# neka-nat/probreg

Hardware: AMD Instinct MI355X
Metric: EM iterations/sec (RigidCPD, N=M=100k fp32) (higher is better)
Workload: dtype f32; 1 GPU; C1 RigidCPD fp32 synthetic N=M=100000 D=3 w=0; window=EM iterations 0..2332 of the registration (state reset after the warm-up steps), collective=none, m=100000, n_local=100000, n_global=100000

## Files before the change

probreg_amd/csrc/cpd.hip:

```cpp
#include <math.h>

#include <algorithm>
#include <cmath>
#include <cstdlib>
#include <cstring>
#include <vector>

#include "cpd_estep.h"
#include "cpd_mstep.h"
#include "cpd_sweeps.h"
#include "morton.h"
#include "small_linalg.h"

namespace {
using prg::block_reduce_store;
using prg::ensure_mompart;
using prg::grid1;
using prg::kBlock;
using prg::kMomComp;
using prg::row_moment_terms;


__global__ __launch_bounds__(kBlock) void k_pack_cloud(const float* __restrict__ in, int64_t n, int dim,
                                                       float4* __restrict__ out, int64_t cap, float pad,
// ... 184 lines not shown
    PRG_HIP(hipMemsetAsync(h->motion.p, 0, 16 * sizeof(unsigned), h->stream));
    return PRG_OK;
}

int morton_permutation(prg_cpd* h, const float* pts_hd, int64_t n, int dim, prg::DevBuf<int>* perm_dev, double* ext2 = nullptr,
                       float* box = nullptr) {
    std::vector<float> host((size_t)n * dim);
    PRG_HIP(hipMemcpy(host.data(), pts_hd, host.size() * sizeof(float), hipMemcpyDefault));
    if (ext2) {
        *ext2 = 0.0;
        for (int k = 0; k < 3; ++k) {
            float lo = INFINITY, hi = -INFINITY;
            for (int64_t i = 0; i < n && k < dim; ++i) {
                lo = std::min(lo, host[(size_t)i * dim + k]);
                hi = std::max(hi, host[(size_t)i * dim + k]);
            }
            if (k >= dim) lo = hi = 0.f;
            *ext2 += (double)(hi - lo) * (double)(hi - lo);
            if (box) {
                box[k] = lo;
                box[3 + k] = hi;
            }
        }
    }
    PRG_HIP(perm_dev->reset(n));
    const std::string& order = prg::cpd_env().spatial_order;
    if (order != "morton" && order != "kd_host") {
        PRG_TRY(prg::ensure_stage(h, (size_t)n * dim * sizeof(float)));
        PRG_HIP(hipMemcpyAsync(h->stage.p, host.data(), host.size() * sizeof(float), hipMemcpyHostToDevice, h->stream));
        return prg::device_kd_order((const float*)h->stage.p, n, dim, perm_dev->p, h->stream);
    }
    const std::vector<int> perm = order == "morton" ? prg::morton_order(host.data(), n, dim) : prg::kd_order(host.data(), n, dim);
    PRG_HIP(hipMemcpy(perm_dev->p, perm.data(), (size_t)n * sizeof(int), hipMemcpyHostToDevice));
    return PRG_OK;
}

}

namespace prg {
int ensure_stage(prg_cpd* h, size_t bytes) {
    if (h->stage.cap >= (int64_t)bytes) return PRG_OK;
    if (h->stage.p) PRG_HIP(hipStreamSynchronize(h->stream));
    PRG_HIP(h->stage.reset((int64_t)bytes));
    return PRG_OK;
}

const CpdEnv& cpd_env() {
    static const CpdEnv env = [] {
        CpdEnv e;
        auto num = [](const char* name, double absent) { const char* v = getenv(name); return v ? atof(v) : absent; };
        auto is_zero = [](const char* name) { const char* v = getenv(name); return v && atoi(v) == 0; };
        e.mfma_seg = getenv("PRG_MFMA_SEG") ? atoi(getenv("PRG_MFMA_SEG")) : 0;
        e.fine_grid_off = is_zero("PRG_MFMA_FINE_GRID");
        e.r_col = num("PRG_ENGINE_RCOL", 0.0);
        e.r_row = num("PRG_ENGINE_RROW", 0.0);
        e.fused_rcol_scale = num("PRG_FUSED_RCOL_SCALE", -1.0);
        e.lean_factor = num("PRG_LEAN_FACTOR", -1.0);
        e.fused_factor = num("PRG_FUSED_FACTOR", -1.0);
        e.owner_off = is_zero("PRG_OWNER_SWEEP");
        e.debug_engine = getenv("PRG_DEBUG_ENGINE") != nullptr;
        if (const char* v = getenv("PRG_SPATIAL_ORDER")) e.spatial_order = v;
        return e;
    }();
    return env;
}

int ensure_engine_state(prg_cpd* h) {
    if (h->eng_dev.p) return PRG_OK;
    PRG_HIP(h->eng_host.ensure(1, kMailboxFlags));
    h->eng_host_dev = h->eng_host.dev;
    PRG_HIP(h->eng_dev.reset(1));
    PRG_HIP(hipMemsetAsync(h->eng_dev.p, 0, sizeof(EngineState), h->stream));
    h->eng_work = h->eng_dev.p->work;
    h->tsum_local = h->eng_dev.p->tsum;
    return PRG_OK;
}
}

extern "C" {

int prg_cpd_create(prg_cpd** out, int device, void* hip_stream) {
    PRG_REQUIRE(out != nullptr, PRG_ERR_INVALID, "prg_cpd_create: out is NULL");
    int count = 0;
    PRG_HIP(hipGetDeviceCount(&count));
    PRG_REQUIRE(device >= 0 && device < count, PRG_ERR_INVALID, "prg_cpd_create: device %d out of range (%d devices)",
                device, count);
    prg::DeviceGuard g(device);
    PRG_REQUIRE(g.ok, PRG_ERR_HIP, "prg_cpd_create: hipSetDevice(%d) failed", device);
    prg_cpd* h = new (std::nothrow) prg_cpd();
    PRG_REQUIRE(h != nullptr, PRG_ERR_NOMEM, "prg_cpd_create: out of host memory");
    h->device = device;
    h->stream = (hipStream_t)hip_stream;
    if (const char* eng = getenv("PRG_DENSE_ENGINE")) h->dense_engine = std::max(0, std::min(2, atoi(eng)));
    if (const char* eng = getenv("PRG_SPARSE_ENGINE")) h->sparse_engine = std::max(0, std::min(2, atoi(eng)));
    if (const char* eng = getenv("PRG_RESID_SWEEP")) h->resid_sweep = atoi(eng) != 0;
    const hipError_t e = h->state.reset(PRG_NMOMENTS + PRG_NPARAMS);
    if (e != hipSuccess) {
        delete h;
        prg::set_error("prg_cpd_create: device allocation failed: %s", hipGetErrorString(e));
        return PRG_ERR_HIP;
    }
    h->moments = h->state.p;
    h->params = h->state.p + PRG_NMOMENTS;
    k_zero_doubles<<<1, 64, 0, h->stream>>>(h->state.p, PRG_NMOMENTS + PRG_NPARAMS);
    *out = h;
    return PRG_OK;
// ... 505 lines not shown
```

probreg_amd/csrc/cpd_estep.hip:

```cpp
#include <math.h>

#include <algorithm>
#include <cmath>

#include "cpd_estep.h"
#include "cpd_sweeps.h"

namespace {
using prg::block_reduce_store;
using prg::grid1;
using prg::kBlock;
using prg::kMomComp;
using prg::row_moment_terms;

constexpr double kLog2e = 1.4426950408889634;

constexpr int kRedBlock = 1024;
__global__ __launch_bounds__(kRedBlock) void k_reduce_partials(const double* __restrict__ part, int nblk, int ncomp,
                                                               double* __restrict__ out, int off) {
    __shared__ double sh[32][33];
    const int c = threadIdx.x & 31, slice = threadIdx.x >> 5;
    double s = 0.0;
    if (c < ncomp)
        for (int b = slice; b < nblk; b += 32) s += part[(int64_t)b * ncomp + c];
// ... 822 lines not shown
    *out = L;
    return PRG_OK;
}
}

namespace {
int ensure_estep_buffers(prg_cpd* h, const EstepLayout& L) {
    PRG_HIP(h->colpart.ensure(L.colpart_elems, L.colpart_elems));
    PRG_HIP(h->rowpart.ensure(L.rowpart_elems, L.rowpart_elems));
    PRG_HIP(h->mompart.ensure(L.mompart_elems, L.mompart_elems));
    if (L.use_queue) PRG_TRY(prg::prepare_queues(h));
    if (L.wgcount_elems > h->wg_cap()) {
        if (h->wgcount.p) PRG_HIP(hipStreamSynchronize(h->stream));
        PRG_HIP(h->wgcount.reset(2 * L.wgcount_elems));
    }
    return PRG_OK;
}

int transform_source(prg_cpd* h, int slot) {
    const double* disp = h->bcpd ? h->W.p : nullptr;
    if (h->nonrigid) PRG_TRY(prg::nonrigid_displacement(h, &disp));
    k_transform_linear<<<(unsigned)prg::ceil_div(h->M, kBlock), kBlock, 0, h->stream>>>(
        h->src4.p, h->z4.p, h->M, h->params, h->motion.p, slot, h->zmeta.p, h->srcw.p, disp, h->zchunk.p);
    return PRG_OK;
}

struct EstepEngines {
    bool use_mfma = false, row_mfma = false;
    bool first = false;
    bool fine = false;
    bool row_lean = false;
    bool fused = false;
    bool col_launched = false;
};

void fill_engine_args(prg_cpd* h, const EstepLayout& L, int slot, EngineArgs* out) {
    const CpdEnv& env = prg::cpd_env();
    EngineArgs ea;
    ea.ext2 = std::max(h->sext2, h->text2);
    ea.r_col_bound = env.r_col > 0.0 ? env.r_col : h->dense_bound > 0.0 ? h->dense_bound : prg::engine_col_bound(h->M, h->N);
    ea.r_col_bound_fused = ea.r_col_bound * fused_lower_bound_scale(L.allow_resid);
    ea.r_row_bound = env.r_row > 0.0 ? env.r_row : prg::engine_row_bound(h->M, h->N, true);
    ea.r_row_bound_full = env.r_row > 0.0 ? env.r_row : prg::engine_row_bound(h->M, h->N, false);
    ea.streamed_col = (double)h->M;
    ea.streamed_row = (double)h->N;
    h->q_first_col = first_queue_unit(ea.r_col_bound, h->N, h->M);
    h->q_first_row = first_queue_unit(ea.r_row_bound, h->M, h->N);
    ea.owned_col = (double)h->N;
    ea.owned_row = (double)h->M;
    ea.work = h->eng_work;
    ea.tsum = h->tsum_local;
    ea.dim = h->D;
    ea.lean_factor = h->lean_factor >= 0.0 ? h->lean_factor : env.lean_factor >= 0.0 ? env.lean_factor : kLeanFactor;
    ea.fused_allowed = L.allow_fused ? 1 : 0;
    ea.resid_allowed = L.allow_resid ? 1 : 0;
    ea.fused_factor = env.fused_factor >= 0.0 ? env.fused_factor : h->fused_factor;
    ea.reset = h->eng.reset ? 1 : 0;
    for (int k = 0; k < 6; ++k) ea.tbox[k] = h->tbox[k];
    ea.slot = slot;
    ea.have_colmin = h->have_colmin ? 1 : 0;
    ea.forced = h->dense_engine >= 2 ? 1 : 0;
    ea.seq = (unsigned)h->estep_count;
    ea.dev = &h->eng_dev.p->decision;
    ea.host = h->eng_host_dev;
    *out = ea;
}

int decide_engines(prg_cpd* h, const EstepLayout& L, int slot, bool cull_seed, hipEvent_t* ev, EstepEngines* out) {
    EstepEngines d;
    *out = d;
    if (!L.mfma_possible || h->eng.mfma_off) {
        if (ev) PRG_HIP(hipEventRecord(ev[1], h->stream));
        return PRG_OK;
    }
    PRG_TRY(prg::ensure_engine_state(h));
    EngineArgs ea;
    fill_engine_args(h, L, slot, &ea);
    h->eng.reset = false;
    prg::launch_chunk_meta_bbox(h, &ea);
    if (ev) PRG_HIP(hipEventRecord(ev[1], h->stream));
    auto seg_col = [&]() { return h->eng.grid_fine && L.seg_col_fine ? L.seg_col_fine : prg::cpd_env().mfma_seg; };
    const bool pred = h->eng.pred_col != 0, pred_fused = L.allow_fused && h->eng.pred_fused != 0;
    const bool vector_grid = !L.use_queue && !L.use_owner;
    if (pred_fused)
        prg::launch_fused_mfma(h, seg_col(), !h->have_colmin, false, ea.dev);
    else if (pred)
        prg::launch_colpass_mfma(h, seg_col(), !h->have_colmin, false, ea.dev, h->mfma_stream && h->eng.pred_fine == 0 && !h->eng.grid_fine);
    else if (vector_grid)
        prg::launch_colpass_cull(h, L.SA, L.segA, cull_seed, ea.dev, L.allow_resid);
    PRG_HIP(hipGetLastError());
    volatile EngineDecision* mb = h->eng_host.p;
    hipError_t werr;
    const bool got = prg::wait_mailbox(&mb->seq, ea.seq, h->stream, &werr);
    PRG_HIP(werr);
    PRG_REQUIRE(got, PRG_ERR_HIP, "prg_cpd_estep: the engine decision never reached the host");
    d.use_mfma = mb->col != 0;
    d.first = mb->first != 0;
    d.row_mfma = mb->row != 0;
    d.fine = mb->fine != 0;
    d.row_lean = d.row_mfma && mb->lean != 0;
    d.fused = L.allow_fused && mb->fused != 0;
    if (!mb->dense) h->eng.mfma_off = true;
    h->eng.grid_fine = !d.first && (double)mb->r_col < 0.9 * (double)h->M;
    if (prg::cpd_env().debug_engine)
        fprintf(stderr, "[engine] sigma2 %.4e nk*ext2 %.1f pairs per owned point col %.0f (bound %.0f) row %.0f (bound %.0f) motion %.3e cmax %.3e nk*width %.1f "
                        "nk*far2 %.1f have_colmin %d -> col %d (first %d, launched ahead: %s) row %d fine %d\n",
                (double)mb->sigma2, (double)mb->nk_ext2, (double)mb->r_col, ea.r_col_bound, (double)mb->r_row, ea.r_row_bound,
                (double)mb->motion, (double)mb->cmax,
                (double)mb->nk_width, (double)mb->nk_far2, (int)h->have_colmin, (int)d.use_mfma, (int)d.first,
                pred == d.use_mfma ? "yes" : "NO", (int)d.row_mfma, (int)d.fine);
    if (pred_fused)
        d.col_launched = d.fused;
    else if (pred)
        d.col_launched = d.use_mfma && !d.fused;
    else
        d.col_launched = !d.use_mfma && vector_grid;
    h->eng.pred_col = d.use_mfma ? 1 : 0;
    h->eng.pred_fine = d.fine ? 1 : 0;
    h->eng.pred_fused = d.fused ? 1 : 0;
    if (!d.col_launched && d.fused) {
        prg::launch_fused_mfma(h, seg_col(), d.first, d.fine, ea.dev);
        d.col_launched = true;
    } else if (!d.col_launched && d.use_mfma) {
        prg::launch_colpass_mfma(h, seg_col(), d.first, d.fine, ea.dev, h->mfma_stream && !d.fine && !h->eng.grid_fine);
        d.col_launched = true;
    }
    *out = d;
    return PRG_OK;
}

struct ColumnPass {
    bool owner = false, queue = false;
};
int column_pass(prg_cpd* h, const EstepLayout& L, const EstepEngines& d, bool resid, bool cull_seed, ColumnPass* out) {
    ColumnPass cp;
    cp.owner = !d.col_launched && resid && L.use_owner;
    cp.queue = !d.col_launched && L.use_queue && !cp.owner;
    if (d.col_launched) {
    } else if (cp.owner)
        prg::launch_colpass_owner(h, cull_seed, L.PO);
    else if (cp.queue)
        PRG_TRY(prg::launch_colpass_queue(h, cull_seed, h->qcol_live ? 0 : h->q_first_col, resid));
    else if (L.use_cull)
        prg::launch_colpass_cull(h, L.SA, L.segA, cull_seed, nullptr, resid);
    else if (L.ra < 0)
        prg::launch_colpass_scalar(h, L.RA, L.SA, L.segA);
    else
        prg::launch_colpass_packed(h, L.RA, L.SA, L.segA);
    *out = cp;
    return PRG_OK;
}

int finish_estep(prg_cpd* h, double w, bool col_queue, bool row_queue, bool rowacc_valid) {
    PRG_HIP(hipGetLastError());
    if (h->comm) {
        PRG_TRY(prg::comm_all_reduce_f64(h->comm, h->moments, kMomComp, h->stream));
        if (h->nonrigid && rowacc_valid) PRG_TRY(prg::comm_all_reduce_f64(h->comm, h->rowacc.p, 4 * h->Mcap, h->stream));
    }
    h->qcol_live = col_queue;
    h->qrow_live = row_queue;
    h->have_estep = true;
    h->estep_state_live = true;
    h->rowacc_valid = rowacc_valid;
    h->have_colmin = true;
    h->last_w = w;
    return PRG_OK;
}

int single_sweep_tail(prg_cpd* h, const EstepLayout& L, const EstepEngines& d, const ColumnPass& cp, bool resid, double w, int slot,
                      hipEvent_t* ev) {
    const int nblk = (int)prg::ceil_div(h->N, kBlock);
    float* const colmin_g = h->colmin.p + h->Ncap;
    const float* part = reinterpret_cast<const float*>(h->colpart.p);
    if (!resid) {
        k_colfinal_fused<<<nblk, kBlock, 0, h->stream>>>(h->tgt4.p, part, h->mfma_col_planes, h->Ncap, h->N, h->pt1.p, h->params, w, m_over_n(h),
                                                         h->D, h->colmin.p, colmin_g, h->tmeta.p, d.first ? 2 : 1, h->motion.p, slot, h->corig.p,
                                                         h->mompart.p);
// ... 85 lines not shown
```

probreg_amd/csrc/cpd_plan.h:

```cpp
#pragma once
#include <cstddef>
#include <vector>

#include "cpd_buffers.h"
#include "prg_common.h"

struct EngineDecision {
    unsigned seq;
    int col;
    int first;
    int row;
    int fine;
    int dense;
    float sigma2, motion, cmax, nk_ext2, nk_width, nk_far2;
    float r_col, r_row;
    int row_off;
    int lean;
    int fused;
    int pad_;
};
struct EngineState {
    EngineDecision decision;
    unsigned long long work[2];
    double tsum[4];
};
static_assert(offsetof(EngineState, work) == sizeof(EngineDecision), "the 64-bit counters sit right behind the decision (pad_)");
constexpr unsigned kMailboxFlags = hipHostMallocMapped | hipHostMallocCoherent;
struct EngineArgs {
    double ext2;
    double r_col_bound, r_row_bound;
    double r_col_bound_fused;
    double r_row_bound_full;
    double owned_col, owned_row;
    double streamed_col, streamed_row;
    const double* tsum;
    double lean_factor;
    double fused_factor;
    int dim;
    unsigned long long* work;
    float tbox[6];
    int slot, have_colmin, forced, reset;
    int fused_allowed;
    int resid_allowed;
    unsigned seq;
    EngineDecision* dev;
    EngineDecision* host;
};

struct EngineSwitch {
    bool reset = true;
    bool mfma_off = false;
    int pred_col = 1;
    int pred_fine = 0;
    int pred_fused = 0;
    bool grid_fine = false;
};

struct CpdEnv {
    int mfma_seg = 0;
    bool fine_grid_off = false;
    double r_col = 0.0, r_row = 0.0;
    double fused_rcol_scale = -1.0;
    double lean_factor = -1.0, fused_factor = -1.0;
    bool owner_off = false;
    bool debug_engine = false;
    std::string spatial_order;
};

using prg::SweepQueue;

struct prg_comm {
    void* nccl = nullptr;
    int rank = 0, nranks = 1, device = 0;
    bool owned = true;
    int64_t calls = 0;
};

struct prg_cpd : prg::SourceBuffers, prg::TargetBuffers {
    int device = 0;
    hipStream_t stream = nullptr;

    int64_t M = 0, N = 0, Nglobal = 0;
    int D = 0;

    prg::DevBuf<float2> colpart;
    prg::DevBuf<float> rowpart;
    prg::DevBuf<double> mompart;

    prg::DevBuf<double> state;
    double* moments = nullptr;
    double* params = nullptr;

    int r_col = 0, seg_col = 0, r_row = 0, seg_row = 0;

    bool opt_sort_src = true, opt_sort_tgt = true, opt_cull = true;
    prg::DevBuf<int> perm_src;
    prg::DevBuf<int> perm_tgt;
    prg::DevBuf<unsigned> motion;
    bool have_colmin = false;
    bool fused_in_iterate = true;
    bool moments_only = false;
    bool init_rot_orthonormal = true;
    bool resid_sweep = true;
    bool last_estep_fused = false;
    bool rowacc_valid = false;
    int dense_engine = 1;
    double dense_bound = 0.0;
    double* tsum_local = nullptr;
    unsigned long long* eng_work = nullptr;
    int q_first_col = 32, q_first_row = 32;
    EngineSwitch eng;
    prg::DevBuf<EngineState> eng_dev;
    prg::HostBuf<EngineDecision> eng_host;
// ... 71 lines not shown
```

probreg_amd/csrc/cpd_sweeps.h:

```cpp
#pragma once
#include "cpd_plan.h"

namespace prg {
constexpr int kSweepBlock = 256;
constexpr int kColChunk = 8;
constexpr int kRowChunk = 4;
constexpr int kOverRead = 8;

__device__ __forceinline__ float col_offset(float kk, float dmin) {
    const float p = -(kk * dmin);
    return p > 0.f ? __uint_as_float(__float_as_uint(p) - 1u) : 0.f;
}

constexpr int kMfmaOwn = 8;
static_assert(kMfmaWgPoints == 4 * 16 * kMfmaOwn, "cpd_buffers.h sizes the origin arrays per workgroup of the matrix-core sweeps");
__device__ __forceinline__ float col_seed_offset(float kk, float cm, float mo) {
    const float r = __fsqrt_rn(cm);
    const float rl = fmaxf(__fsub_rn(r, mo), 0.f), rh = __fadd_rn(r, mo);
    const float lo = __fmul_rn(rl, rl), hi = __fmul_rn(rh, rh);
    const float nk = -kk;
    const float g = __fmul_rn(nk, __fsub_rn(hi, lo));
    return __fadd_rn(__fmul_rn(nk, lo), fmaxf(__fsub_rn(g, 80.f), 0.f));
}
void launch_colpass_mfma(prg_cpd* h, int S, bool first, bool fine, const EngineDecision* guard, bool stream);
int mfma_stream_planes(int64_t owned_points, int64_t streamed_points);
void launch_chunk_meta_bbox(prg_cpd* h, const EngineArgs* eng);
void launch_fused_mfma(prg_cpd* h, int S, bool first, bool fine, const EngineDecision* guard);
void launch_rowpass_mfma(prg_cpd* h, int S, bool fine, bool lean, bool stream);
int mfma_planes(int64_t owned_points, int64_t streamed_points, int S);
int mfma_chunks_per_seg(int64_t owned_points, int64_t streamed_points, int S);
int mfma_chunks_per_seg_model(int64_t owned_points, int64_t streamed_points);

constexpr int kOwnerWaves = 8;
constexpr int kOwnerMaxPlanes = 32;
constexpr int kOwnerColsPerLane = 1;
int owner_cols_per_lane();
int owner_planes(int64_t owned_points, int64_t streamed_points);
void launch_colpass_owner(prg_cpd* h, bool use_seed, int planes);

constexpr int kQueueTargetUnits = 16384;
constexpr int kQueueMaxUnits = 98304;
constexpr int kQueueWorkgroups = 2048;
int launch_colpass_queue(prg_cpd* h, bool use_seed, int q_init, bool resid = false);
int launch_rowpass_queue(prg_cpd* h, int q_init);
int64_t queue_max_units(int64_t owned_points, int64_t streamed_points);
int prepare_queues(prg_cpd* h);

#ifndef PRG_CULL_EXP
#define PRG_CULL_EXP 48
#endif
constexpr float kCullExp = (float)PRG_CULL_EXP;
void launch_colpass_cull(prg_cpd* h, int S, int seg_len, bool use_seed, const EngineDecision* guard = nullptr, bool resid = false);
inline unsigned char* resid_flags(const prg_cpd* h, int planes) {
    return reinterpret_cast<unsigned char*>(reinterpret_cast<float*>(h->colpart.p) + (int64_t)planes * 6 * h->Ncap);
}
void launch_rowpass_cull(prg_cpd* h, int S, int seg_len);
void launch_colpass_packed(prg_cpd* h, int R, int S, int seg_len);
void launch_rowpass_packed(prg_cpd* h, int R, int S, int seg_len);
void launch_colpass_scalar(prg_cpd* h, int R, int S, int seg_len);
void launch_rowpass_scalar(prg_cpd* h, int R, int S, int seg_len);
}
```

probreg_amd/csrc/cpd_sweeps_mfma.hip:

```cpp
#include <math.h>

#include <algorithm>
#include <map>
#include <mutex>
#include <vector>

#include "cpd_sweeps.h"

namespace {

typedef float f32x4 __attribute__((ext_vector_type(4)));
typedef float f32x2 __attribute__((ext_vector_type(2)));
typedef __bf16 bf16x8 __attribute__((ext_vector_type(8)));

constexpr double kLog2e = 1.4426950408889634;
constexpr int kBlock = prg::kSweepBlock;
constexpr int kOwn = prg::kMfmaOwn;
constexpr int kWgPoints = 4 * 16 * kOwn;
constexpr int kChunk = 256;
constexpr int kChunkTiles = kChunk / 16;
constexpr int kTileBytes = 1024 + 5 * 64;
constexpr int kTileFloats = kTileBytes / 4;

__device__ __forceinline__ float exp2r(float a) { return __builtin_amdgcn_exp2f(a); }
__device__ __forceinline__ float xor_sum(float v) {
    v += __shfl_xor(v, 16, 64);
    v += __shfl_xor(v, 32, 64);
    return v;
}
__device__ __forceinline__ float xor_max(float v) {
    v = fmaxf(v, __shfl_xor(v, 16, 64));
    v = fmaxf(v, __shfl_xor(v, 32, 64));
    return v;
}

struct alignas(32) BoxMeta { float lo[3]; float hi[3]; float aux; float pad; };

__device__ __forceinline__ float box_gap2(const float (&alo)[3], const float (&ahi)[3], const BoxMeta& g) {
    float d2 = 0.f;
#pragma unroll
    for (int k = 0; k < 3; ++k) {
        const float gap = fmaxf(fmaxf(alo[k] - g.hi[k], g.lo[k] - ahi[k]), 0.f);
        d2 = fmaf(gap, gap, d2);
    }
    return d2;
}

__device__ __forceinline__ bool wg_box(const BoxMeta* __restrict__ gmeta, int64_t first_point, int64_t n_points, int lane,
                                       float (&lo)[3], float (&hi)[3]) {
    const int64_t g = first_point / 32 + (lane & 15);
    const bool valid = (g + 1) * 32 <= n_points;
    const BoxMeta m = gmeta[g];
#pragma unroll
    for (int k = 0; k < 3; ++k) {
        lo[k] = valid ? m.lo[k] : INFINITY;
        hi[k] = valid ? m.hi[k] : -INFINITY;
#pragma unroll
        for (int sh = 1; sh < 16; sh <<= 1) {
            lo[k] = fminf(lo[k], __shfl_xor(lo[k], sh, 64));
            hi[k] = fmaxf(hi[k], __shfl_xor(hi[k], sh, 64));
        }
    }
    return hi[0] >= lo[0];
}

struct WaveBox { float lo[3]; float hi[3]; };
__device__ __forceinline__ bool wave_box(const BoxMeta* __restrict__ gmeta, int64_t first_point, int64_t n_points, int lane,
                                         WaveBox& w) {
    const BoxMeta m = gmeta[first_point / 32 + (lane & 3)];
#pragma unroll
    for (int k = 0; k < 3; ++k) {
        float l = m.lo[k], h = m.hi[k];
        l = fminf(l, __shfl_xor(l, 1, 64));
        l = fminf(l, __shfl_xor(l, 2, 64));
        h = fmaxf(h, __shfl_xor(h, 1, 64));
        h = fmaxf(h, __shfl_xor(h, 2, 64));
        w.lo[k] = __uint_as_float(__builtin_amdgcn_readfirstlane(__float_as_uint(l)));
        w.hi[k] = __uint_as_float(__builtin_amdgcn_readfirstlane(__float_as_uint(h)));
    }
    return first_point + 16 * kOwn <= n_points;
}

__device__ __forceinline__ unsigned tiles_of_groups(unsigned g) {
    g = (g | (g << 4)) & 0x0F0Fu;
    g = (g | (g << 2)) & 0x3333u;
    g = (g | (g << 1)) & 0x5555u;
    return g | (g << 1);
}

struct Split3 { __bf16 h, m, l; };
__device__ __forceinline__ Split3 split3(float a) {
    Split3 s;
    s.h = (__bf16)a;
    const float r1 = a - (float)s.h;
    s.m = (__bf16)r1;
    s.l = (__bf16)(r1 - (float)s.m);
    return s;
}
__device__ __forceinline__ bf16x8 slots_streamed(const Split3 s) {
    const __bf16 z = (__bf16)0.f;
    return (bf16x8){s.h, s.h, s.m, s.h, s.l, s.m, z, z};
}
__device__ __forceinline__ bf16x8 slots_owned(const Split3 s) {
    const __bf16 z = (__bf16)0.f;
    return (bf16x8){s.h, s.m, s.h, s.l, s.h, s.m, z, z};
}

__device__ __forceinline__ void stage_point(float* __restrict__ buf, int p, const float4 v, const float4 o, float kk,
                                            bool lean = false) {
    const float dx = v.x - o.x, dy = v.y - o.y, dz = v.z - o.z;
    const float sq = fmaf(dz, dz, fmaf(dy, dy, dx * dx));
    float* tile = buf + (p >> 4) * kTileFloats;
    bf16x8* a = reinterpret_cast<bf16x8*>(tile);
    const int j = p & 15;
    const __bf16 one = (__bf16)1.f, z = (__bf16)0.f;
    a[0 * 16 + j] = slots_streamed(split3(dx));
    a[1 * 16 + j] = slots_streamed(split3(dy));
    a[2 * 16 + j] = slots_streamed(split3(dz));
    a[3 * 16 + j] = (bf16x8){one, one, one, z, z, z, z, z};
    float* f = tile + 256;
    f[j] = fmaf(kk, sq, v.w);
    *reinterpret_cast<float2*>(f + 16 + 2 * j) = make_float2(dx, dy);
    *reinterpret_cast<float2*>(f + 48 + 2 * j) = make_float2(dz, lean ? 1.f : sq);
}

__device__ __forceinline__ bf16x8 owned_operand(int k, float kk, float dx, float dy, float dz, float cst) {
    const float m2 = -2.f * kk;
    if (k == 0) return slots_owned(split3(m2 * dx));
    if (k == 1) return slots_owned(split3(m2 * dy));
    if (k == 2) return slots_owned(split3(m2 * dz));
    const Split3 c = split3(cst);
    const __bf16 z = (__bf16)0.f;
    return (bf16x8){c.h, c.m, c.l, z, z, z, z, z};
}

struct WorkItem { int blk; int c0; int nc; int plane; bool ends_block; };
struct StreamCut { int g; int pmax; unsigned base; unsigned rem; };
__device__ __forceinline__ unsigned sk_start(unsigned w, const StreamCut sc) { return w * sc.base + (w < sc.rem ? w : sc.rem); }
__device__ __forceinline__ WorkItem sk_item(unsigned u, unsigned u_end, unsigned w, unsigned nchunks, const StreamCut sc) {
    WorkItem it;
    const unsigned blk = u / nchunks, c0 = u - blk * nchunks;
    const unsigned left = nchunks - c0, want = u_end - u;
    it.blk = (int)blk;
    it.c0 = (int)c0;
    it.nc = (int)(want < left ? want : left);
    it.ends_block = c0 + (unsigned)it.nc == nchunks;
    const unsigned x = blk * nchunks, big = sc.rem * (sc.base + 1u);
    const unsigned wf = x < big ? x / (sc.base + 1u) : sc.rem + (x - big) / sc.base;
    it.plane = (int)(w - wf);
    return it;
}

template <bool FUSED>
__global__ __launch_bounds__(kBlock) __attribute__((amdgpu_waves_per_eu(3, FUSED ? 3 : 10))) void k_colpass_mfma(
                                                         const float4* __restrict__ tgt4, const float4* __restrict__ z4,
                                                         const BoxMeta* __restrict__ tmeta,
                                                         const BoxMeta* __restrict__ zmeta,
                                                         const BoxMeta* __restrict__ zchunk,
                                                         const float* __restrict__ colmin_prev,
                                                         const float* __restrict__ colmin_g,
                                                         const unsigned* __restrict__ motion, int chunks_per_seg,
                                                         int64_t m_total, int64_t n_total,
                                                         const double* __restrict__ params,
                                                         float2* __restrict__ colpart, int64_t ncap,
                                                         unsigned* __restrict__ wgcount, unsigned long long* __restrict__ work,
                                                         int first, int fine,
                                                         const EngineDecision* __restrict__ guard, const StreamCut sk,
                                                         float4* __restrict__ corig) {
    __shared__ __attribute__((aligned(16))) float stage[2][kChunkTiles * kTileFloats];
    __shared__ unsigned wave_tiles[kBlock / 64];
    if (guard) {
        const bool fused_wanted = guard->col == 1 && guard->fused == 1;
        if (FUSED ? !fused_wanted : (guard->col != 1 || fused_wanted)) return;
        fine = guard->fine;
    }
    const int lane = threadIdx.x & 63, wv = __builtin_amdgcn_readfirstlane((int)(threadIdx.x >> 6));
    const float kk = (float)(-kLog2e / (2.0 * params[13]));
    const float mo = __uint_as_float(*motion);
    const int nchunks = (int)((m_total + kChunk - 1) / kChunk), nblocks = (int)((n_total + kWgPoints - 1) / kWgPoints);
    const int sk_g = FUSED ? 0 : sk.g, sk_pmax = sk.pmax;
    unsigned unit = sk_g ? sk_start(blockIdx.x, sk) : 0u;
    const unsigned unit_end = sk_g ? sk_start(blockIdx.x + 1u, sk) : 0u;
    for (;;) {
    WorkItem item;
    if (sk_g) {
        item = sk_item(unit, unit_end, blockIdx.x, (unsigned)nchunks, sk);
    } else {
        item.blk = (int)blockIdx.x;
        item.c0 = (int)blockIdx.y * chunks_per_seg;
        item.nc = (item.c0 + chunks_per_seg < nchunks ? item.c0 + chunks_per_seg : nchunks) - item.c0;
        item.plane = blockIdx.y;
        item.ends_block = false;
    }
    const int64_t n0wg = (int64_t)item.blk * kWgPoints, n0 = n0wg + wv * (16 * kOwn);
    float lo[3], hi[3];
    float4 o;
    float thr = INFINITY;
    float thr_w = INFINITY;
    WaveBox wb;
    bool wave_cull = wave_box(tmeta, n0, n_total, lane, wb) && !first && fine;
    if (n0wg + kWgPoints <= n_total && wg_box(tmeta, n0wg, n_total, lane, lo, hi)) {
        o = make_float4(0.5f * (lo[0] + hi[0]), 0.5f * (lo[1] + hi[1]), 0.5f * (lo[2] + hi[2]), 0.f);
        if (!first) {
            float cm = colmin_g[n0wg / 32 + (lane & 15)];
            float cw = __shfl(cm, 4 * wv + (lane & 3), 64);
            cw = fmaxf(cw, __shfl_xor(cw, 1, 64));
            cw = fmaxf(cw, __shfl_xor(cw, 2, 64));
#pragma unroll
            for (int sh = 1; sh < 16; sh <<= 1) cm = fmaxf(cm, __shfl_xor(cm, sh, 64));
            const float r = sqrtf(cm) + mo, rw = sqrtf(cw) + mo;
            thr = r * r * 1.00001f + (-prg::kCullExp) / kk;
            thr_w = rw * rw * 1.00001f + (-prg::kCullExp) / kk;
        }
    } else {
        o = tgt4[n0wg];
        o.w = 0.f;
        wave_cull = false;
#pragma unroll
        for (int q = 0; q < 3; ++q) { lo[q] = -INFINITY; hi[q] = INFINITY; }
    }
    const int k = lane >> 4, j = lane & 15;
    bf16x8 bx[kOwn];
    float s[kOwn], tm[kOwn], off[FUSED ? 1 : kOwn];
    f32x2 uxy[FUSED ? kOwn : 1], uze[FUSED ? kOwn : 1];
#pragma unroll
    for (int t = 0; t < kOwn; ++t) {
        const float4 x = tgt4[n0 + 16 * t + j];
        const float xx = x.x - o.x, xy = x.y - o.y, xz = x.z - o.z;
        const float xsq = fmaf(xz, xz, fmaf(xy, xy, xx * xx));
        const float offt = first ? 0.f : prg::col_seed_offset(kk, colmin_prev[n0 + 16 * t + j], mo);
        if (!FUSED) off[t] = offt;
        bx[t] = owned_operand(k, kk, xx, xy, xz, fmaf(kk, xsq, offt));
        s[t] = 0.f;
        tm[t] = -INFINITY;
        if (FUSED) uxy[t] = uze[t] = (f32x2){0.f, 0.f};
    }
    unsigned tiles_done = 0;
    const int64_t c0 = item.c0;
    const int nc = item.nc;
    const BoxMeta cm = zchunk[c0 + (lane < nc ? lane : nc - 1)];
    unsigned long long mask = __ballot(lane < nc && !(box_gap2(lo, hi, cm) > thr));
    if (mask) {
        int cur = __builtin_ctzll(mask);
        mask &= mask - 1;
        float4 ra = z4[(c0 + cur) * kChunk + threadIdx.x];
        ra.w = 0.f;
        BoxMeta gm = zmeta[wave_cull ? (c0 + cur) * 8 + (lane & 7) : 0];
        stage_point(stage[0], threadIdx.x, ra, o, kk);
        __syncthreads();
        for (int bsel = 0;; bsel ^= 1) {
            const float* __restrict__ buf = stage[bsel];
            unsigned tmask = 0xFFFFu;
            if (wave_cull)
                tmask = tiles_of_groups((unsigned)__ballot(lane < 8 && !(box_gap2(wb.lo, wb.hi, gm) > thr_w)) & 0xFFu);
            const int nxt = mask ? __builtin_ctzll(mask) : -1;
            mask &= mask - 1;
            if (nxt >= 0) {
                ra = z4[(c0 + nxt) * kChunk + threadIdx.x];
                ra.w = 0.f;
                if (wave_cull) gm = zmeta[(c0 + nxt) * 8 + (lane & 7)];
            }
            tiles_done += __popc(tmask);
            auto tile_step = [&](f32x4& d, const float* __restrict__ tb, const bf16x8 a1, const f32x4 cz, const bf16x8 a1n,
                                 const f32x4 czn) {
                f32x2 xy0, xy1, xy2, xy3, zs0, zs1, zs2, zs3;
                if (FUSED) {
                    const f32x4 a01 = *reinterpret_cast<const f32x4*>(tb + 272 + 8 * k), a23 = *reinterpret_cast<const f32x4*>(tb + 276 + 8 * k),
                                b01 = *reinterpret_cast<const f32x4*>(tb + 304 + 8 * k), b23 = *reinterpret_cast<const f32x4*>(tb + 308 + 8 * k);
                    xy0 = (f32x2){a01[0], a01[1]}; xy1 = (f32x2){a01[2], a01[3]}; xy2 = (f32x2){a23[0], a23[1]}; xy3 = (f32x2){a23[2], a23[3]};
                    zs0 = (f32x2){b01[0], b01[1]}; zs1 = (f32x2){b01[2], b01[3]}; zs2 = (f32x2){b23[0], b23[1]}; zs3 = (f32x2){b23[2], b23[3]};
                }
#pragma unroll
                for (int u = 0; u < kOwn; ++u) {
                    const f32x4 dn = u + 1 < kOwn ? __builtin_amdgcn_mfma_f32_16x16x32_bf16(a1, bx[u + 1], cz, 0, 0, 0)
                                                  : __builtin_amdgcn_mfma_f32_16x16x32_bf16(a1n, bx[0], czn, 0, 0, 0);
                    tm[u] = fmaxf(fmaxf(tm[u], d[0]), d[1]);
                    tm[u] = fmaxf(fmaxf(tm[u], d[2]), d[3]);
                    const float q0 = exp2r(d[0]), q1 = exp2r(d[1]), q2 = exp2r(d[2]), q3 = exp2r(d[3]);
                    s[u] += (q0 + q1) + (q2 + q3);
                    if (FUSED) {
                        const f32x2 s0 = {q0, q0}, s1 = {q1, q1}, s2 = {q2, q2}, s3 = {q3, q3};
                        uxy[u] = __builtin_elementwise_fma(s3, xy3, __builtin_elementwise_fma(s2, xy2, __builtin_elementwise_fma(s1, xy1, __builtin_elementwise_fma(s0, xy0, uxy[u]))));
                        uze[u] = __builtin_elementwise_fma(s3, zs3, __builtin_elementwise_fma(s2, zs2, __builtin_elementwise_fma(s1, zs1, __builtin_elementwise_fma(s0, zs0, uze[u]))));
                    }
                    d = dn;
                }
            };
            if (tmask == 0xFFFFu) {
                bf16x8 a1 = reinterpret_cast<const bf16x8*>(buf)[lane];
                f32x4 cz = *reinterpret_cast<const f32x4*>(buf + 256 + 4 * k);
                f32x4 d = __builtin_amdgcn_mfma_f32_16x16x32_bf16(a1, bx[0], cz, 0, 0, 0);
                for (int t = 0; t < kChunkTiles; ++t) {
                    const float* __restrict__ tn = buf + (t + 1 < kChunkTiles ? t + 1 : t) * kTileFloats;
                    const bf16x8 a1n = reinterpret_cast<const bf16x8*>(tn)[lane];
                    const f32x4 czn = *reinterpret_cast<const f32x4*>(tn + 256 + 4 * k);
                    tile_step(d, buf + t * kTileFloats, a1, cz, a1n, czn);
                    a1 = a1n;
                    cz = czn;
                }
            } else if (tmask) {
                int t = __builtin_ctz(tmask);
                tmask &= tmask - 1;
                bf16x8 a1 = reinterpret_cast<const bf16x8*>(buf + t * kTileFloats)[lane];
                f32x4 cz = *reinterpret_cast<const f32x4*>(buf + t * kTileFloats + 256 + 4 * k);
                f32x4 d = __builtin_amdgcn_mfma_f32_16x16x32_bf16(a1, bx[0], cz, 0, 0, 0);
                for (;;) {
                    const bool more = tmask != 0;
                    const int t2 = more ? __builtin_ctz(tmask) : t;
                    tmask &= tmask - 1;
                    const float* __restrict__ tn = buf + t2 * kTileFloats;
                    const bf16x8 a1n = reinterpret_cast<const bf16x8*>(tn)[lane];
                    const f32x4 czn = *reinterpret_cast<const f32x4*>(tn + 256 + 4 * k);
                    tile_step(d, buf + t * kTileFloats, a1, cz, a1n, czn);
// ... 307 lines not shown
        }
    __syncthreads();
    if (threadIdx.x != 0) return;
    float box[6];
#pragma unroll
    for (int q = 0; q < 6; ++q) {
        float v = sh[0][q];
        for (int w = 1; w < kBlock / 64; ++w) v = q < 3 ? fminf(v, sh[w][q]) : fmaxf(v, sh[w][q]);
        box[q] = v;
        stat[8 + q] = __float_as_uint(v);
    }
    if (!eng.dev) return;
    const double sigma2 = params[13], nk = kLog2e / (2.0 * sigma2);
    const double mo = __uint_as_float(stat[eng.slot]), cmax = __uint_as_float(stat[4 + (eng.slot ^ 1)]), r = sqrt(cmax);
    const double width = r >= mo ? 4.0 * r * mo : (r + mo) * (r + mo);
    const bool ok = sigma2 > 0.0 && isfinite(sigma2);
    const EngineDecision prev = *eng.dev;
    float r_col = eng.reset ? (float)eng.streamed_col : prev.r_col, r_row = eng.reset ? (float)eng.streamed_row : prev.r_row;
    int row_off = eng.reset ? 0 : prev.row_off;
    const unsigned long long tc = eng.work[0], tr = eng.work[1];
    eng.work[0] = 0ull;
    eng.work[1] = 0ull;
    if (tc && !eng.reset) r_col = (float)((double)tc * 2048.0 / eng.owned_col);
    if (tr && !eng.reset) r_row = (float)((double)tr * 2048.0 / eng.owned_row);

    const bool lean_ok = eng.tsum && eng.tsum[3] > 0.0 && sigma2 * (double)eng.dim * eng.lean_factor * eng.owned_col >= eng.tsum[3];
    if (prev.fused && tc && !eng.reset) r_row = (float)((double)r_col * eng.owned_col / eng.owned_row);
    const bool fused_ok = eng.tsum && eng.tsum[3] > 0.0 && sigma2 * (double)eng.dim * eng.fused_factor * eng.owned_col >= eng.tsum[3];
    const bool fused_try = eng.fused_allowed && fused_ok && !row_off;
    bool dense = ok && (eng.forced || r_col >= (fused_try ? eng.r_col_bound_fused : eng.r_col_bound));
    if (dense && !eng.forced && eng.fused_allowed && eng.resid_allowed && !fused_try && !(r_col >= 0.6 * eng.streamed_col)) dense = false;
    if (!fused_try && !(r_row >= (lean_ok ? eng.r_row_bound : eng.r_row_bound_full))) row_off = 1;
    double far2 = 0.0;
#pragma unroll
    for (int k = 0; k < 3; ++k) {
        const double a = fabs((double)eng.tbox[3 + k] - (double)box[k]), b = fabs((double)box[3 + k] - (double)eng.tbox[k]);
        far2 += fmax(a, b) * fmax(a, b);
    }
    const bool first = dense && !eng.have_colmin && isfinite(far2) && nk * far2 < 110.0;
    const bool col = first || (dense && eng.have_colmin && isfinite(cmax) && nk * width < 150.0);
    const bool row = dense && (eng.forced || !row_off);
    const bool lean = row && lean_ok;
    EngineDecision d;
    d.seq = eng.seq;
    d.col = col ? 1 : 0;
    d.first = first ? 1 : 0;
    d.row = row ? 1 : 0;
    d.fine = nk * eng.ext2 > 200.0 * (prg::kCullExp / 127.0) ? 1 : 0;
    d.dense = dense ? 1 : 0;
    d.sigma2 = (float)sigma2; d.motion = (float)mo; d.cmax = (float)cmax;
    d.nk_ext2 = (float)(nk * eng.ext2); d.nk_width = (float)(nk * width); d.nk_far2 = (float)(nk * far2);
    d.r_col = r_col; d.r_row = r_row; d.row_off = row_off; d.lean = lean ? 1 : 0;
    d.fused = eng.fused_allowed && col && row && fused_ok ? 1 : 0;
    *eng.dev = d;
    EngineDecision* hm = eng.host;
    hm->col = d.col; hm->first = d.first; hm->row = d.row; hm->fine = d.fine; hm->dense = d.dense;
    hm->sigma2 = d.sigma2; hm->motion = d.motion; hm->cmax = d.cmax;
    hm->nk_ext2 = d.nk_ext2; hm->nk_width = d.nk_width; hm->nk_far2 = d.nk_far2;
    hm->r_col = d.r_col; hm->r_row = d.r_row; hm->row_off = d.row_off; hm->lean = d.lean; hm->fused = d.fused;
    __threadfence_system();
    __hip_atomic_store(&hm->seq, d.seq, __ATOMIC_RELEASE, __HIP_MEMORY_SCOPE_SYSTEM);
}

}

namespace prg {

static double mfma_dense_makespan(int64_t blocks, int64_t chunks, int64_t cps, double over) {
    const int64_t segs = ceil_div(chunks, cps), rem = chunks - (segs - 1) * cps;
    std::vector<double> slot(768, 0.0);
    auto later = [](double a, double b) { return a > b; };
    double end = 0.0;
    for (int64_t y = 0; y < segs; ++y) {
        const double d = (double)(y + 1 < segs ? cps : rem) + over;
        for (int64_t x = 0; x < blocks; ++x) {
            std::pop_heap(slot.begin(), slot.end(), later);
            const double t = slot.back() + d;
            slot.back() = t;
            std::push_heap(slot.begin(), slot.end(), later);
            end = std::max(end, t);
        }
    }
    return end;
}

int mfma_chunks_per_seg(int64_t owned_points, int64_t streamed_points, int S) {
    const int64_t chunks = ceil_div(streamed_points, kChunk);
    if (S <= 0) {
        const int64_t blocks = ceil_div(owned_points, kWgPoints);
        static std::mutex mu;
        static std::map<std::pair<int64_t, int64_t>, int> memo;
        static const bool old_model = getenv("PRG_MFMA_SEG_MODEL") && atoi(getenv("PRG_MFMA_SEG_MODEL")) == 4;
        std::lock_guard<std::mutex> lock(mu);
        const auto key = std::make_pair(blocks, chunks);
        const auto hit = memo.find(key);
        if (hit != memo.end()) {
            S = hit->second;
        } else {
            double best = 1e30;
            S = 1;
            for (int64_t cand = 4; cand <= 32; ++cand) {
                const int64_t cps = ceil_div(chunks, std::min<int64_t>(cand, chunks));
                if (cps > 64) continue;
                const int64_t segs = ceil_div(chunks, cps);
                const double cost = old_model ? (double)ceil_div(blocks * segs, (int64_t)768) * (double)cps
                                              : mfma_dense_makespan(blocks, chunks, cps, 0.15);
                if (cost < best * 0.999) {
                    best = cost;
                    S = (int)cand;
                }
            }
            memo[key] = S;
// ... 24 lines not shown
    return (int)ceil_div(ceil_div(streamed_points, kChunk), cps);
}

void launch_chunk_meta(prg_cpd* h, const float* gmeta, int64_t cap, float* cmeta) {
    const int64_t nchunk = cap / kChunk;
    k_chunk_meta<<<(unsigned)ceil_div(nchunk, kBlock), kBlock, 0, h->stream>>>(reinterpret_cast<const BoxMeta*>(gmeta), nchunk,
                                                                             reinterpret_cast<BoxMeta*>(cmeta));
}

void launch_chunk_meta_bbox(prg_cpd* h, const EngineArgs* eng) {
    EngineArgs none;
    none.dev = nullptr;
    none.host = nullptr;
    k_chunk_meta_bbox<<<1, kBlock, 0, h->stream>>>(reinterpret_cast<const BoxMeta*>(h->zmeta.p), h->Mcap / kChunk,
                                                  reinterpret_cast<BoxMeta*>(h->zchunk.p), h->z4.p, h->M, h->motion.p, h->params,
                                                  eng ? *eng : none);
}

constexpr int kStreamSlots = 768;
static int64_t stream_workgroups(int64_t blocks, int64_t chunks) {
    const int64_t units = blocks * chunks;
    return kStreamSlots * ceil_div(units, (int64_t)kStreamSlots * 64);
}
int mfma_stream_planes(int64_t owned_points, int64_t streamed_points) {
    static const bool off = getenv("PRG_MFMA_STREAM") && atoi(getenv("PRG_MFMA_STREAM")) == 0;
    const int64_t blocks = ceil_div(owned_points, kWgPoints), chunks = ceil_div(streamed_points, kChunk);
    if (off || blocks * chunks < 4 * (int64_t)kStreamSlots || blocks * chunks >= (int64_t)1 << 31) return 0;
    static thread_local int64_t last_blocks = -1, last_chunks = -1;
    static thread_local int last_planes = 0;
    if (blocks != last_blocks || chunks != last_chunks) {
        const int64_t units = blocks * chunks, g = stream_workgroups(blocks, chunks), base = units / g, rem = units % g;
        auto holder = [&](int64_t x) { return x < rem * (base + 1) ? x / (base + 1) : rem + (x - rem * (base + 1)) / base; };
        int64_t most = 0;
        for (int64_t b = 0; b < blocks; ++b) most = std::max(most, holder((b + 1) * chunks - 1) - holder(b * chunks) + 1);
        last_blocks = blocks;
        last_chunks = chunks;
        last_planes = (int)most;
    }
    return last_planes <= 48 ? last_planes : 0;
}

static StreamCut stream_cut(int planes, int64_t blocks, int64_t chunks) {
    StreamCut c = {0, 0, 0u, 0u};
    if (planes > 0) {
        const int64_t units = blocks * chunks, g = stream_workgroups(blocks, chunks);
        c.g = (int)g;
        c.pmax = planes;
        c.base = (unsigned)(units / g);
        c.rem = (unsigned)(units % g);
    }
    return c;
}

void launch_colpass_mfma(prg_cpd* h, int S, bool first, bool fine, const EngineDecision* guard, bool stream) {
    const int cps = mfma_chunks_per_seg(h->N, h->M, S);
    const int sp = stream ? mfma_stream_planes(h->N, h->M) : 0;
    const int64_t nblocks = ceil_div(h->N, kWgPoints);
    dim3 grid((unsigned)nblocks, (unsigned)ceil_div(ceil_div(h->M, kChunk), cps));
    h->mfma_col_planes = sp ? sp : (int)grid.y;
    const StreamCut cut = stream_cut(sp, nblocks, ceil_div(h->M, kChunk));
    if (sp) grid = dim3((unsigned)cut.g, 1);
    k_colpass_mfma<false><<<grid, kBlock, 0, h->stream>>>(h->tgt4.p, h->z4.p, reinterpret_cast<const BoxMeta*>(h->tmeta.p),
                                                   reinterpret_cast<const BoxMeta*>(h->zmeta.p),
                                                   reinterpret_cast<const BoxMeta*>(h->zchunk.p), h->colmin.p, h->colmin.p + h->Ncap,
                                                   h->motion.p + ((h->estep_count - 1) & 1), cps, h->M, h->N, h->params,
                                                   h->colpart.p, h->Ncap, h->wgcount.p, h->eng_work, first ? 1 : 0, fine ? 1 : 0, guard,
                                                   cut, nullptr);
    h->wg_col = nblocks * h->mfma_col_planes;
    h->wg_col_pairs = 128.0 * 16.0;
    h->dense_pairs_col = 0.0;
}

void launch_fused_mfma(prg_cpd* h, int S, bool first, bool fine, const EngineDecision* guard) {
    const int cps = mfma_chunks_per_seg(h->N, h->M, S);
    const int64_t nblocks = ceil_div(h->N, kWgPoints);
    dim3 grid((unsigned)nblocks, (unsigned)ceil_div(ceil_div(h->M, kChunk), cps));
    h->mfma_col_planes = (int)grid.y;
    const StreamCut none = {0, 0, 0u, 0u};
    k_colpass_mfma<true><<<grid, kBlock, 0, h->stream>>>(h->tgt4.p, h->z4.p, reinterpret_cast<const BoxMeta*>(h->tmeta.p),
                                                         reinterpret_cast<const BoxMeta*>(h->zmeta.p),
                                                         reinterpret_cast<const BoxMeta*>(h->zchunk.p), h->colmin.p, h->colmin.p + h->Ncap,
                                                         h->motion.p + ((h->estep_count - 1) & 1), cps, h->M, h->N, h->params,
                                                         h->colpart.p, h->Ncap, h->wgcount.p, h->eng_work, first ? 1 : 0, fine ? 1 : 0, guard,
                                                         none, h->corig.p);
    h->wg_col = nblocks * h->mfma_col_planes;
    h->wg_col_pairs = 128.0 * 16.0;
    h->dense_pairs_col = 0.0;
}

void launch_rowpass_mfma(prg_cpd* h, int S, bool fine, bool lean, bool stream) {
    const int cps = mfma_chunks_per_seg(h->M, h->N, S);
    const int sp = stream && lean ? mfma_stream_planes(h->M, h->N) : 0;
    const int64_t nblocks = ceil_div(h->M, kWgPoints);
    dim3 grid((unsigned)nblocks, (unsigned)ceil_div(ceil_div(h->N, kChunk), cps));
    h->mfma_row_planes = sp ? sp : (int)grid.y;
    const StreamCut cut = stream_cut(sp, nblocks, ceil_div(h->N, kChunk));
    if (sp) grid = dim3((unsigned)cut.g, 1);
    unsigned char* rowflag = reinterpret_cast<unsigned char*>(h->rowpart.p + (int64_t)h->mfma_row_planes * 5 * h->Mcap);
    launch_chunk_meta(h, h->tmeta.p, h->Ncap, h->tchunk.p);
    auto kernel = sp ? k_rowpass_mfma<true, true> : lean ? k_rowpass_mfma<true, false> : k_rowpass_mfma<false, false>;
    kernel<<<grid, kBlock, 0, h->stream>>>(h->z4.p, h->tgt4.p, reinterpret_cast<const BoxMeta*>(h->zmeta.p),
                                           reinterpret_cast<const BoxMeta*>(h->tmeta.p), reinterpret_cast<const BoxMeta*>(h->tchunk.p), cps,
                                           h->N, h->M, h->params, h->rowpart.p, h->Mcap, h->rorig.p, rowflag, h->wgcount.p + h->wg_cap(),
                                           h->eng_work + 1, fine ? 1 : 0, cut);
    h->wg_row = nblocks * h->mfma_row_planes;
    h->wg_row_pairs = 128.0 * 16.0;
    h->dense_pairs_row = 0.0;
}

}
```

Before: 10010 EM iterations/s.

## Deal streamed chunks round-robin across MFMA column-pass planes when culling is sparse

Adds a 'deal' mode to the MFMA column/fused pass. Chunks are assigned to grid-y planes with a stride of gridDim.y instead of as contiguous segments, so culled (surviving) chunk work spreads evenly across workgroups rather than piling up on the few planes near the spatial neighbourhood. The mode is chosen on device when the surviving column pairs fall below a fraction of M, and it is relayed through the mailbox for the next predicted launch. A tail-workgroup bounding box is also added so partial blocks can cull too, which costs extra shuffles and carries some risk of strided, less-local chunk loads.

```diff
diff --git a/probreg_amd/csrc/cpd.hip b/probreg_amd/csrc/cpd.hip
--- a/probreg_amd/csrc/cpd.hip
+++ b/probreg_amd/csrc/cpd.hip
@@ -260,6 +260,8 @@
         auto is_zero = [](const char* name) { const char* v = getenv(name); return v && atoi(v) == 0; };
         e.mfma_seg = getenv("PRG_MFMA_SEG") ? atoi(getenv("PRG_MFMA_SEG")) : 0;
         e.fine_grid_off = is_zero("PRG_MFMA_FINE_GRID");
+        e.mfma_deal = getenv("PRG_MFMA_DEAL") ? (atoi(getenv("PRG_MFMA_DEAL")) != 0 ? 1 : 0) : -1;
+        e.mfma_deal_below = num("PRG_MFMA_DEAL_BELOW", 0.9);
         e.r_col = num("PRG_ENGINE_RCOL", 0.0);
         e.r_row = num("PRG_ENGINE_RROW", 0.0);
         e.fused_rcol_scale = num("PRG_FUSED_RCOL_SCALE", -1.0);
diff --git a/probreg_amd/csrc/cpd_estep.hip b/probreg_amd/csrc/cpd_estep.hip
--- a/probreg_amd/csrc/cpd_estep.hip
+++ b/probreg_amd/csrc/cpd_estep.hip
@@ -898,6 +898,8 @@
     ea.tsum = h->tsum_local;
     ea.dim = h->D;
     ea.lean_factor = h->lean_factor >= 0.0 ? h->lean_factor : env.lean_factor >= 0.0 ? env.lean_factor : kLeanFactor;
+    ea.deal_mode = env.mfma_deal;
+    ea.deal_below = env.mfma_deal_below;
     ea.fused_allowed = L.allow_fused ? 1 : 0;
     ea.resid_allowed = L.allow_resid ? 1 : 0;
     ea.fused_factor = env.fused_factor >= 0.0 ? env.fused_factor : h->fused_factor;
@@ -929,9 +931,9 @@
     const bool pred = h->eng.pred_col != 0, pred_fused = L.allow_fused && h->eng.pred_fused != 0;
     const bool vector_grid = !L.use_queue && !L.use_owner;
     if (pred_fused)
-        prg::launch_fused_mfma(h, seg_col(), !h->have_colmin, false, ea.dev);
+        prg::launch_fused_mfma(h, seg_col(), !h->have_colmin, false, h->eng.deal != 0, ea.dev);
     else if (pred)
-        prg::launch_colpass_mfma(h, seg_col(), !h->have_colmin, false, ea.dev, h->mfma_stream && h->eng.pred_fine == 0 && !h->eng.grid_fine);
+        prg::launch_colpass_mfma(h, seg_col(), !h->have_colmin, false, h->eng.deal != 0, ea.dev, h->mfma_stream && h->eng.pred_fine == 0 && !h->eng.grid_fine);
     else if (vector_grid)
         prg::launch_colpass_cull(h, L.SA, L.segA, cull_seed, ea.dev, L.allow_resid);
     PRG_HIP(hipGetLastError());
@@ -964,11 +966,12 @@
     h->eng.pred_col = d.use_mfma ? 1 : 0;
     h->eng.pred_fine = d.fine ? 1 : 0;
     h->eng.pred_fused = d.fused ? 1 : 0;
+    h->eng.deal = mb->deal;
     if (!d.col_launched && d.fused) {
-        prg::launch_fused_mfma(h, seg_col(), d.first, d.fine, ea.dev);
+        prg::launch_fused_mfma(h, seg_col(), d.first, d.fine, h->eng.deal != 0, ea.dev);
         d.col_launched = true;
     } else if (!d.col_launched && d.use_mfma) {
-        prg::launch_colpass_mfma(h, seg_col(), d.first, d.fine, ea.dev, h->mfma_stream && !d.fine && !h->eng.grid_fine);
+        prg::launch_colpass_mfma(h, seg_col(), d.first, d.fine, h->eng.deal != 0, ea.dev, h->mfma_stream && !d.fine && !h->eng.grid_fine);
         d.col_launched = true;
     }
     *out = d;
diff --git a/probreg_amd/csrc/cpd_plan.h b/probreg_amd/csrc/cpd_plan.h
--- a/probreg_amd/csrc/cpd_plan.h
+++ b/probreg_amd/csrc/cpd_plan.h
@@ -17,14 +17,15 @@
     int row_off;
     int lean;
     int fused;
-    int pad_;
+    int deal;
 };
 struct EngineState {
     EngineDecision decision;
     unsigned long long work[2];
     double tsum[4];
 };
-static_assert(offsetof(EngineState, work) == sizeof(EngineDecision), "the 64-bit counters sit right behind the decision (pad_)");
+static_assert(offsetof(EngineState, work) == sizeof(EngineDecision) && sizeof(EngineDecision) % 8 == 0,
+              "the 64-bit counters sit right behind the decision");
 constexpr unsigned kMailboxFlags = hipHostMallocMapped | hipHostMallocCoherent;
 struct EngineArgs {
     double ext2;
@@ -40,6 +41,8 @@
     unsigned long long* work;
     float tbox[6];
     int slot, have_colmin, forced, reset;
+    int deal_mode;
+    double deal_below;
     int fused_allowed;
     int resid_allowed;
     unsigned seq;
@@ -54,11 +57,14 @@
     int pred_fine = 0;
     int pred_fused = 0;
     bool grid_fine = false;
+    int deal = 0;
 };
 
 struct CpdEnv {
     int mfma_seg = 0;
     bool fine_grid_off = false;
+    int mfma_deal = -1;
+    double mfma_deal_below = 0.9;
     double r_col = 0.0, r_row = 0.0;
     double fused_rcol_scale = -1.0;
     double lean_factor = -1.0, fused_factor = -1.0;
diff --git a/probreg_amd/csrc/cpd_sweeps.h b/probreg_amd/csrc/cpd_sweeps.h
--- a/probreg_amd/csrc/cpd_sweeps.h
+++ b/probreg_amd/csrc/cpd_sweeps.h
@@ -22,10 +22,10 @@
     const float g = __fmul_rn(nk, __fsub_rn(hi, lo));
     return __fadd_rn(__fmul_rn(nk, lo), fmaxf(__fsub_rn(g, 80.f), 0.f));
 }
-void launch_colpass_mfma(prg_cpd* h, int S, bool first, bool fine, const EngineDecision* guard, bool stream);
+void launch_colpass_mfma(prg_cpd* h, int S, bool first, bool fine, bool deal, const EngineDecision* guard, bool stream);
 int mfma_stream_planes(int64_t owned_points, int64_t streamed_points);
 void launch_chunk_meta_bbox(prg_cpd* h, const EngineArgs* eng);
-void launch_fused_mfma(prg_cpd* h, int S, bool first, bool fine, const EngineDecision* guard);
+void launch_fused_mfma(prg_cpd* h, int S, bool first, bool fine, bool deal, const EngineDecision* guard);
 void launch_rowpass_mfma(prg_cpd* h, int S, bool fine, bool lean, bool stream);
 int mfma_planes(int64_t owned_points, int64_t streamed_points, int S);
 int mfma_chunks_per_seg(int64_t owned_points, int64_t streamed_points, int S);
diff --git a/probreg_amd/csrc/cpd_sweeps_mfma.hip b/probreg_amd/csrc/cpd_sweeps_mfma.hip
--- a/probreg_amd/csrc/cpd_sweeps_mfma.hip
+++ b/probreg_amd/csrc/cpd_sweeps_mfma.hip
@@ -59,6 +59,29 @@
         for (int sh = 1; sh < 16; sh <<= 1) {
             lo[k] = fminf(lo[k], __shfl_xor(lo[k], sh, 64));
             hi[k] = fmaxf(hi[k], __shfl_xor(hi[k], sh, 64));
+        }
+    }
+    return hi[0] >= lo[0];
+}
+
+__device__ __forceinline__ bool wg_box_tail(const BoxMeta* __restrict__ gmeta, const float4* __restrict__ pts, int64_t first_point,
+                                            int64_t n_points, int lane, float (&lo)[3], float (&hi)[3]) {
+    wg_box(gmeta, first_point, n_points, lane, lo, hi);
+    const int64_t tail = n_points / 32 * 32;
+    if (tail < n_points && tail >= first_point) {
+        const int64_t i = tail + (lane & 31);
+        const float4 p = pts[i < n_points ? i : tail];
+        const float c[3] = {p.x, p.y, p.z};
+#pragma unroll
+        for (int k = 0; k < 3; ++k) {
+            float l = c[k], h = c[k];
+#pragma unroll
+            for (int sh = 1; sh < 32; sh <<= 1) {
+                l = fminf(l, __shfl_xor(l, sh, 64));
+                h = fmaxf(h, __shfl_xor(h, sh, 64));
+            }
+            lo[k] = fminf(lo[k], l);
+            hi[k] = fmaxf(hi[k], h);
         }
     }
     return hi[0] >= lo[0];
@@ -164,7 +187,7 @@
                                                          const double* __restrict__ params,
                                                          float2* __restrict__ colpart, int64_t ncap,
                                                          unsigned* __restrict__ wgcount, unsigned long long* __restrict__ work,
-                                                         int first, int fine,
+                                                         int first, int fine, int deal,
                                                          const EngineDecision* __restrict__ guard, const StreamCut sk,
                                                          float4* __restrict__ corig) {
     __shared__ __attribute__((aligned(16))) float stage[2][kChunkTiles * kTileFloats];
@@ -173,6 +196,7 @@
         const bool fused_wanted = guard->col == 1 && guard->fused == 1;
         if (FUSED ? !fused_wanted : (guard->col != 1 || fused_wanted)) return;
         fine = guard->fine;
+        deal = guard->deal;
     }
     const int lane = threadIdx.x & 63, wv = __builtin_amdgcn_readfirstlane((int)(threadIdx.x >> 6));
     const float kk = (float)(-kLog2e / (2.0 * params[13]));
@@ -187,8 +211,13 @@
         item = sk_item(unit, unit_end, blockIdx.x, (unsigned)nchunks, sk);
     } else {
         item.blk = (int)blockIdx.x;
-        item.c0 = (int)blockIdx.y * chunks_per_seg;
-        item.nc = (item.c0 + chunks_per_seg < nchunks ? item.c0 + chunks_per_seg : nchunks) - item.c0;
+        if (deal) {
+            item.c0 = (int)blockIdx.y;
+            item.nc = item.c0 < nchunks ? (nchunks - item.c0 + (int)gridDim.y - 1) / (int)gridDim.y : 0;
+        } else {
+            item.c0 = (int)blockIdx.y * chunks_per_seg;
+            item.nc = (item.c0 + chunks_per_seg < nchunks ? item.c0 + chunks_per_seg : nchunks) - item.c0;
+        }
         item.plane = blockIdx.y;
         item.ends_block = false;
     }
@@ -199,8 +228,14 @@
     float thr_w = INFINITY;
     WaveBox wb;
     bool wave_cull = wave_box(tmeta, n0, n_total, lane, wb) && !first && fine;
-    if (n0wg + kWgPoints <= n_total && wg_box(tmeta, n0wg, n_total, lane, lo, hi)) {
-        o = make_float4(0.5f * (lo[0] + hi[0]), 0.5f * (lo[1] + hi[1]), 0.5f * (lo[2] + hi[2]), 0.f);
+    const bool whole = n0wg + kWgPoints <= n_total;
+    if (whole ? wg_box(tmeta, n0wg, n_total, lane, lo, hi) : wg_box_tail(tmeta, tgt4, n0wg, n_total, lane, lo, hi)) {
+        if (whole) {
+            o = make_float4(0.5f * (lo[0] + hi[0]), 0.5f * (lo[1] + hi[1]), 0.5f * (lo[2] + hi[2]), 0.f);
+        } else {
+            o = tgt4[n0wg];
+            o.w = 0.f;
+        }
         if (!first) {
             float cm = colmin_g[n0wg / 32 + (lane & 15)];
             float cw = __shfl(cm, 4 * wv + (lane & 3), 64);
@@ -236,16 +271,17 @@
         if (FUSED) uxy[t] = uze[t] = (f32x2){0.f, 0.f};
     }
     unsigned tiles_done = 0;
-    const int64_t c0 = item.c0;
+    const int c0 = item.c0, cstride = !sk_g && deal ? (int)gridDim.y : 1;
+    auto chunk_of = [&](int i) { return (int64_t)(c0 + i * cstride); };
     const int nc = item.nc;
-    const BoxMeta cm = zchunk[c0 + (lane < nc ? lane : nc - 1)];
+    const BoxMeta cm = zchunk[chunk_of(lane < nc ? lane : nc > 0 ? nc - 1 : 0)];
     unsigned long long mask = __ballot(lane < nc && !(box_gap2(lo, hi, cm) > thr));
     if (mask) {
         int cur = __builtin_ctzll(mask);
         mask &= mask - 1;
-        float4 ra = z4[(c0 + cur) * kChunk + threadIdx.x];
+        float4 ra = z4[chunk_of(cur) * kChunk + threadIdx.x];
         ra.w = 0.f;
-        BoxMeta gm = zmeta[wave_cull ? (c0 + cur) * 8 + (lane & 7) : 0];
+        BoxMeta gm = zmeta[wave_cull ? chunk_of(cur) * 8 + (lane & 7) : 0];
         stage_point(stage[0], threadIdx.x, ra, o, kk);
         __syncthreads();
         for (int bsel = 0;; bsel ^= 1) {
@@ -256,9 +292,9 @@
             const int nxt = mask ? __builtin_ctzll(mask) : -1;
             mask &= mask - 1;
             if (nxt >= 0) {
-                ra = z4[(c0 + nxt) * kChunk + threadIdx.x];
+                ra = z4[chunk_of(nxt) * kChunk + threadIdx.x];
                 ra.w = 0.f;
-                if (wave_cull) gm = zmeta[(c0 + nxt) * 8 + (lane & 7)];
+                if (wave_cull) gm = zmeta[chunk_of(nxt) * 8 + (lane & 7)];
             }
             tiles_done += __popc(tmask);
             auto tile_step = [&](f32x4& d, const float* __restrict__ tb, const bf16x8 a1, const f32x4 cz, const bf16x8 a1n,
@@ -672,12 +708,13 @@
     d.nk_ext2 = (float)(nk * eng.ext2); d.nk_width = (float)(nk * width); d.nk_far2 = (float)(nk * far2);
     d.r_col = r_col; d.r_row = r_row; d.row_off = row_off; d.lean = lean ? 1 : 0;
     d.fused = eng.fused_allowed && col && row && fused_ok ? 1 : 0;
+    d.deal = eng.deal_mode >= 0 ? eng.deal_mode : (!first && (double)r_col < eng.deal_below * eng.streamed_col ? 1 : 0);
     *eng.dev = d;
     EngineDecision* hm = eng.host;
     hm->col = d.col; hm->first = d.first; hm->row = d.row; hm->fine = d.fine; hm->dense = d.dense;
     hm->sigma2 = d.sigma2; hm->motion = d.motion; hm->cmax = d.cmax;
     hm->nk_ext2 = d.nk_ext2; hm->nk_width = d.nk_width; hm->nk_far2 = d.nk_far2;
-    hm->r_col = d.r_col; hm->r_row = d.r_row; hm->row_off = d.row_off; hm->lean = d.lean; hm->fused = d.fused;
+    hm->r_col = d.r_col; hm->r_row = d.r_row; hm->row_off = d.row_off; hm->lean = d.lean; hm->fused = d.fused; hm->deal = d.deal;
     __threadfence_system();
     __hip_atomic_store(&hm->seq, d.seq, __ATOMIC_RELEASE, __HIP_MEMORY_SCOPE_SYSTEM);
 }
@@ -808,7 +845,7 @@
     return c;
 }
 
-void launch_colpass_mfma(prg_cpd* h, int S, bool first, bool fine, const EngineDecision* guard, bool stream) {
+void launch_colpass_mfma(prg_cpd* h, int S, bool first, bool fine, bool deal, const EngineDecision* guard, bool stream) {
     const int cps = mfma_chunks_per_seg(h->N, h->M, S);
     const int sp = stream ? mfma_stream_planes(h->N, h->M) : 0;
     const int64_t nblocks = ceil_div(h->N, kWgPoints);
@@ -820,14 +857,14 @@
                                                    reinterpret_cast<const BoxMeta*>(h->zmeta.p),
                                                    reinterpret_cast<const BoxMeta*>(h->zchunk.p), h->colmin.p, h->colmin.p + h->Ncap,
                                                    h->motion.p + ((h->estep_count - 1) & 1), cps, h->M, h->N, h->params,
-                                                   h->colpart.p, h->Ncap, h->wgcount.p, h->eng_work, first ? 1 : 0, fine ? 1 : 0, guard,
+                                                   h->colpart.p, h->Ncap, h->wgcount.p, h->eng_work, first ? 1 : 0, fine ? 1 : 0, deal ? 1 : 0, guard,
                                                    cut, nullptr);
     h->wg_col = nblocks * h->mfma_col_planes;
     h->wg_col_pairs = 128.0 * 16.0;
     h->dense_pairs_col = 0.0;
 }
 
-void launch_fused_mfma(prg_cpd* h, int S, bool first, bool fine, const EngineDecision* guard) {
+void launch_fused_mfma(prg_cpd* h, int S, bool first, bool fine, bool deal, const EngineDecision* guard) {
     const int cps = mfma_chunks_per_seg(h->N, h->M, S);
     const int64_t nblocks = ceil_div(h->N, kWgPoints);
     dim3 grid((unsigned)nblocks, (unsigned)ceil_div(ceil_div(h->M, kChunk), cps));
@@ -837,7 +874,7 @@
                                                          reinterpret_cast<const BoxMeta*>(h->zmeta.p),
                                                          reinterpret_cast<const BoxMeta*>(h->zchunk.p), h->colmin.p, h->colmin.p + h->Ncap,
                                                          h->motion.p + ((h->estep_count - 1) & 1), cps, h->M, h->N, h->params,
-                                                         h->colpart.p, h->Ncap, h->wgcount.p, h->eng_work, first ? 1 : 0, fine ? 1 : 0, guard,
+                                                         h->colpart.p, h->Ncap, h->wgcount.p, h->eng_work, first ? 1 : 0, fine ? 1 : 0, deal ? 1 : 0, guard,
                                                          none, h->corig.p);
     h->wg_col = nblocks * h->mfma_col_planes;
     h->wg_col_pairs = 128.0 * 16.0;
```

Result: faster. 10150 EM iterations/s (median of 6 runs) (+1.4%).
